# TravisWheelerLab/BATH

Hardware: AMD Instinct MI355X
Metric: DP Gcells/s + residues/s through bathsearch pipeline at 1/2/4/8 MI355X (higher is better)
Workload: dtype u8/i16 integer scores (SSV: exact binary16), f32 Forward

## Files before the change

### bath_amd/csrc/bath_profile.hip

```cpp
#include <atomic>
#include <cctype>
#include <cmath>
#include <cstring>

#include "bath_common.hpp"
#include "host_model.hpp"

using namespace bath;

namespace bath {

static const double kLog2 = 0.69314718055994529;

double gumbel_surv(double x, double mu, double lambda) {
  double ey = -std::exp(-lambda * (x - mu));
  if (std::fabs(ey) < 5e-9) return -ey;
  return 1.0 - std::exp(ey);
}
double gumbel_invsurv(double p, double mu, double lambda) {
  double lp = (p < 5e-9) ? (std::pow(p, p) - 1) / p : std::log(-1. * std::log(1 - p));
  return mu - lp / lambda;
}
double exp_surv(double x, double mu, double lambda) { return (x < mu) ? 1.0 : std::exp(-lambda * (x - mu)); }

// ... 100 lines not shown

extern "C" void bath_hip_finalize(bath_hip_ctx *ctx) {
  if (!ctx) return;
  bath::g_ctx_total.fetch_sub(1);
  if (ctx->internal) bath::g_ctx_internal.fetch_sub(1);
  (void)hipSetDevice(ctx->device);
  (void)hipStreamSynchronize(ctx->stream);
  delete ctx->lane_pool; ctx->lane_pool = nullptr;
  for (bath_hip_ctx *lane : ctx->lanes) bath_hip_finalize(lane);
  ctx->lanes.clear();
  if (ctx->ev_lanes) (void)hipEventDestroy(ctx->ev_lanes);
  if (ctx->aux) { bath_hip_finalize(ctx->aux); ctx->aux = nullptr; }
  if (ctx->aux2) { bath_hip_finalize(ctx->aux2); ctx->aux2 = nullptr; }
  if (ctx->aux3) { bath_hip_finalize(ctx->aux3); ctx->aux3 = nullptr; }
  for (auto &b : ctx->scratch) b.release();
  for (auto &b : ctx->stage) b.release();
  ctx->results_pinned.release();
  for (auto e : ctx->ev_pool) (void)hipEventDestroy(e);
  for (auto e : ctx->span_events) (void)hipEventDestroy(e);
  if (ctx->ev_fork) (void)hipEventDestroy(ctx->ev_fork);
  if (ctx->ev_join) (void)hipEventDestroy(ctx->ev_join);
  if (ctx->copy_stream) (void)hipStreamDestroy(ctx->copy_stream);
  if (ctx->side_stream) (void)hipStreamDestroy(ctx->side_stream);
  (void)hipStreamDestroy(ctx->stream);
  delete ctx;
}

extern "C" int bath_hip_trim(bath_hip_ctx *ctx) {
  if (!ctx) return BATH_EINVAL;
  BATH_HIP_TRY(ctx, hipSetDevice(ctx->device));
  BATH_HIP_TRY(ctx, hipStreamSynchronize(ctx->stream));
  delete ctx->lane_pool; ctx->lane_pool = nullptr;
  for (bath_hip_ctx *lane : ctx->lanes) bath_hip_finalize(lane);
  ctx->lanes.clear();
  if (ctx->aux) { bath_hip_finalize(ctx->aux); ctx->aux = nullptr; }
  if (ctx->aux2) { bath_hip_finalize(ctx->aux2); ctx->aux2 = nullptr; }
  if (ctx->aux3) { bath_hip_finalize(ctx->aux3); ctx->aux3 = nullptr; }
  if (ctx->copy_stream) { (void)hipStreamSynchronize(ctx->copy_stream); (void)hipStreamDestroy(ctx->copy_stream); ctx->copy_stream = nullptr; }
  if (ctx->side_stream) {
    (void)hipStreamSynchronize(ctx->side_stream); (void)hipStreamDestroy(ctx->side_stream); ctx->side_stream = nullptr;
    if (ctx->ev_fork) { (void)hipEventDestroy(ctx->ev_fork); ctx->ev_fork = nullptr; }
    if (ctx->ev_join) { (void)hipEventDestroy(ctx->ev_join); ctx->ev_join = nullptr; }
  }
  ctx->fs_std_orfs.clear(); ctx->fs_std_pool = nullptr; ctx->fs_keep_xoff.clear(); ctx->fs_regions_all.clear();
  ctx->d_records = nullptr; ctx->n_records = 0;
  return BATH_OK;
}

extern "C" const char *bath_hip_last_error(const bath_hip_ctx *ctx) { return ctx ? ctx->err.c_str() : "no context"; }

extern "C" int bath_hip_synchronize(bath_hip_ctx *ctx) {
  BATH_HIP_TRY(ctx, hipSetDevice(ctx->device));
  BATH_HIP_TRY(ctx, hipStreamSynchronize(ctx->stream));
  return BATH_OK;
}

extern "C" void *bath_hip_stream(bath_hip_ctx *ctx) { return (void *)ctx->stream; }
extern "C" int bath_hip_kernel_times(bath_hip_ctx *ctx, int max, bath_kernel_time *out) {
  if (!ctx || !out) return 0;
  int n = 0;
  for (const bath_hip_ctx *c : {(const bath_hip_ctx *)ctx, (const bath_hip_ctx *)ctx->aux, (const bath_hip_ctx *)ctx->aux2, (const bath_hip_ctx *)ctx->aux3}) {
    if (!c) continue;
    for (const bath::KernelSpan &k : c->spans) {
      float ms = 0.f;
      if (hipEventSynchronize(k.b) != hipSuccess || hipEventElapsedTime(&ms, k.a, k.b) != hipSuccess) continue;
      int i = 0;
      while (i < n && out[i].name != k.name) i++;
      if (i == n) { if (n == max) continue; out[n++] = bath_kernel_time{k.name, 0.f, 0, 0.0, 0.0}; }
      out[i].ms += ms; out[i].launches++; out[i].cells += k.cells; out[i].bytes += k.bytes;
    }
  }
  return n;
}
extern "C" int bath_hip_set_fs_serial(bath_hip_ctx *ctx, int on) {
  if (!ctx) return BATH_EINVAL;
  ctx->fs_serial = on < 0 ? -1 : (on ? 1 : 0);
  return BATH_OK;
}

extern "C" int bath_hip_set_fs_strict(bath_hip_ctx *ctx, int on) {
  if (!ctx) return BATH_EINVAL;
  ctx->fs_strict = on ? 1 : 0;
  if (!on && ctx->aux3) { bath_hip_finalize(ctx->aux3); ctx->aux3 = nullptr; }
  for (bath_hip_ctx *l : ctx->lanes) l->fs_strict = ctx->fs_strict;
  return BATH_OK;
}

extern "C" int bath_hip_set_fwd_group(bath_hip_ctx *ctx, int mode) {
  if (!ctx) return BATH_EINVAL;
  if (mode < 0 || mode > 2) { ctx->set_error("bath_hip_set_fwd_group: mode must be 0, 1 or 2"); return BATH_EINVAL; }
  ctx->fwd_group = mode;
  for (bath_hip_ctx *l : ctx->lanes) l->fwd_group = mode;
  return BATH_OK;
}

extern "C" int bath_hip_set_fs_odds(bath_hip_ctx *ctx, int on) {
  if (!ctx) return BATH_EINVAL;
  ctx->fs_odds = on ? 1 : 0;
  for (bath_hip_ctx *l : ctx->lanes) l->fs_odds = ctx->fs_odds;
  return BATH_OK;
}

extern "C" int bath_hip_set_fs5_odds(bath_hip_ctx *ctx, int on) {
  if (!ctx) return BATH_EINVAL;
  ctx->fs5_odds = on ? 1 : 0;
  for (bath_hip_ctx *l : ctx->lanes) l->fs5_odds = ctx->fs5_odds;
  return BATH_OK;
}

extern "C" int bath_hip_set_fs_ensemble(bath_hip_ctx *ctx, int mode) {
  if (!ctx) return BATH_EINVAL;
  if (mode != BATH_ENSEMBLE_SERIAL && mode != BATH_ENSEMBLE_STREAMS_HOST && mode != BATH_ENSEMBLE_STREAMS_DEVICE) { ctx->set_error("bath_hip_set_fs_ensemble: unknown mode " + std::to_string(mode)); return BATH_EINVAL; }
  ctx->fs_ensemble = mode;
  for (bath_hip_ctx *l : ctx->lanes) l->fs_ensemble = mode;
  return BATH_OK;
}

extern "C" int bath_hip_set_std_ensemble(bath_hip_ctx *ctx, int mode) {
  if (!ctx) return BATH_EINVAL;
  if (mode != BATH_ENSEMBLE_SERIAL && mode != BATH_ENSEMBLE_STREAMS_HOST && mode != BATH_ENSEMBLE_STREAMS_DEVICE) { ctx->set_error("bath_hip_set_std_ensemble: unknown mode " + std::to_string(mode)); return BATH_EINVAL; }
  ctx->std_ensemble = mode;
  for (bath_hip_ctx *l : ctx->lanes) l->std_ensemble = mode;
  if (ctx->aux) ctx->aux->std_ensemble = mode;
  return BATH_OK;
}

extern "C" int bath_hip_std_ensemble_counters(bath_hip_ctx *ctx, int64_t *serial_fallbacks, int64_t *twin_fallbacks, int64_t *kernel_regions) {
  if (!ctx) return BATH_EINVAL;
  int64_t s = 0, t = 0, k = 0;
  for (const bath_hip_ctx *c : {(const bath_hip_ctx *)ctx, (const bath_hip_ctx *)ctx->aux}) {
    if (!c) continue;
    s += c->std_ens_serial_fallbacks.load(); t += c->std_ens_twin_fallbacks.load(); k += c->std_ens_kernel_regions.load();
  }
  if (serial_fallbacks) *serial_fallbacks = s;
  if (twin_fallbacks) *twin_fallbacks = t;
  if (kernel_regions) *kernel_regions = k;
  return BATH_OK;
}

extern "C" int bath_hip_fs_ensemble_counters(bath_hip_ctx *ctx, int64_t *bound_fallbacks, int64_t *overflow_fallbacks, int64_t *matrix_bytes_kept) {
  if (!ctx) return BATH_EINVAL;
  int64_t b = 0, o = 0, k = 0;
  for (const bath_hip_ctx *c : {(const bath_hip_ctx *)ctx, (const bath_hip_ctx *)ctx->aux2}) {
    if (!c) continue;
    b += c->fs_ens_bound_fallbacks.load(); o += c->fs_ens_overflow_fallbacks.load(); k += c->fs_ens_bytes_kept.load();
  }
  if (bound_fallbacks) *bound_fallbacks = b;
  if (overflow_fallbacks) *overflow_fallbacks = o;
  if (matrix_bytes_kept) *matrix_bytes_kept = k;
  return BATH_OK;
}

extern "C" int bath_selftest_compute_units(const bath_hip_ctx *ctx) { return ctx ? ctx->prop.multiProcessorCount : 0; }


extern "C" void bath_hip_oprofile_destroy(bath_hip_oprofile *om) {
  if (!om) return;
  for (void *p : {(void *)om->d_emit, (void *)om->d_ssv, (void *)om->d_msv, (void *)om->d_rb, (void *)om->d_rw, (void *)om->d_tw, (void *)om->d_rf, (void *)om->d_tf,
                  (void *)om->d_bias_eo, (void *)om->d_compo_terms, (void *)om->d_vit_rw, (void *)om->d_vit_tw2, (void *)om->d_vit_rank, (void *)om->lt.d_tjb, (void *)om->lt.d_xwmove, (void *)om->lt.d_pmove,
                  (void *)om->lt.d_nullsc, (void *)om->lt.d_lt1, (void *)om->lt.d_lt2, (void *)om->lt.d_p1, (void *)om->d_cons, (void *)om->d_msc, (void *)om->d_tsc, (void *)om->d_rfb, (void *)om->d_tfb})
    if (p) (void)hipFree(p);
  for (void *p : om->retired) (void)hipFree(p);
  delete om;
}

extern "C" int bath_hip_oprofile_set_consensus(bath_hip_oprofile *om, const char *consensus) {
  if (!om || !consensus) return BATH_EINVAL;
  bath_hip_ctx *ctx = om->ctx;
  static const char syms[] = "ACDEFGHIKLMNPQRSTVWY-BJZOUX*~";
  om->consensus.assign((size_t)om->M + 2, ' ');
  om->cons_digital.assign((size_t)om->M + 1, 255);
  for (int k = 1; k <= om->M && consensus[k]; k++) {
    om->consensus[(size_t)k] = consensus[k];
    const char *q = std::strchr(syms, std::toupper((unsigned char)consensus[k]));
    if (q) om->cons_digital[(size_t)k] = (uint8_t)(q - syms);
  }
  if (!om->d_cons) BATH_HIP_TRY(ctx, hipMalloc(&om->d_cons, (size_t)om->M + 1));
  BATH_HIP_TRY(ctx, hipMemcpy(om->d_cons, om->cons_digital.data(), (size_t)om->M + 1, hipMemcpyHostToDevice));
  return BATH_OK;
}

extern "C" int bath_hip_oprofile_M(const bath_hip_oprofile *om) { return om->M; }

extern "C" int bath_hip_oprofile_convert(bath_hip_ctx *ctx, const bath_profile *gm, bath_hip_oprofile **ret) {
  *ret = nullptr;
  const int M = gm->M;
  if (M < 1) { ctx->set_error("profile has no nodes"); return BATH_EINVAL; }
  BATH_HIP_TRY(ctx, hipSetDevice(ctx->device));
  const size_t W = (size_t)M + 1;
  auto msc = [&](int k, int x) { return gm->rsc[(size_t)x * W * 2 + 2 * k]; };
  auto tsc = [&](int k, int s) { return gm->tsc[(size_t)k * 8 + s]; };
  enum { MM, IM, DM, BM, MD, DD, MI, II };

  bath_hip_oprofile *om = new bath_hip_oprofile();
  { static std::atomic<uint64_t> next_uid{1}; om->uid = next_uid.fetch_add(1); }
  om->ctx = ctx; om->M = M; om->max_length = gm->max_length; om->nj = gm->nj; om->L0 = gm->L;
  std::memcpy(om->evparam, gm->evparam, sizeof om->evparam);
  std::memcpy(om->compo, gm->compo, sizeof om->compo);

  float maxsc = 0.0f;
  for (int x = 0; x < 20; x++)
    for (size_t i = 0; i < W * 2; i++) maxsc = std::max(maxsc, gm->rsc[(size_t)x * W * 2 + i]);
  om->scale_b = (float)(3.0 / kLog2);
  om->base_b = 190;
  om->bias_b = cost_u8(om->scale_b, (float)(-1.0 * maxsc));
  om->rb.assign((size_t)kKp * W, 255);
  for (int x = 0; x < kKp; x++)
    for (int k = 1; k <= M; k++) om->rb[x * W + k] = cost_u8_biased(om->scale_b, om->bias_b, msc(k, x));
  om->tbm_b = cost_u8(om->scale_b, logf(2.0f / ((float)M * (float)(M + 1))));
  om->tec_b = cost_u8(om->scale_b, logf(0.5f));

  om->scale_w = (float)(500.0 / kLog2);
  om->base_w = 12000;
  om->rw.assign((size_t)kKp * W, -32768);
  for (int x = 0; x < kKp; x++)
    for (int k = 1; k <= M; k++) om->rw[x * W + k] = score_i16(om->scale_w, msc(k, x));
  om->tw.assign(W * 8, -32768);
  for (int k = 1; k <= M; k++) {
    int16_t *t = &om->tw[(size_t)k * 8];
    for (int s : {BM, MM, IM, DM}) t[s] = std::min<int16_t>(score_i16(om->scale_w, tsc(k - 1, s)), 0);
    for (int s : {MD, MI}) t[s] = (k < M) ? std::min<int16_t>(score_i16(om->scale_w, tsc(k, s)), 0) : (int16_t)-32768;
    t[II] = (k < M) ? std::min<int16_t>(score_i16(om->scale_w, tsc(k, II)), -1) : (int16_t)-32768;
    t[DD] = (k < M) ? score_i16(om->scale_w, tsc(k, DD)) : (int16_t)-32768;
  }
  om->xw_E[0] = score_i16(om->scale_w, gm->xsc[0][0]);
  om->xw_E[1] = score_i16(om->scale_w, gm->xsc[0][1]);
  int ddb = -32768;
  for (int k = 2; k < M - 1; k++)
    ddb = std::max(ddb, (int)score_i16(om->scale_w, tsc(k, DD)) + (int)score_i16(om->scale_w, tsc(k + 1, DM)) -
                            (int)score_i16(om->scale_w, tsc(k + 1, BM)));
  om->ddbound_w = (int16_t)ddb;

  om->rf.assign((size_t)kKp * W, 0.f);
  for (int x = 0; x < kKp; x++)
    for (int k = 1; k <= M; k++) om->rf[x * W + k] = expf(msc(k, x));
  om->tf.assign(W * 8, 0.f);
  for (int k = 1; k <= M; k++) {
    float *t = &om->tf[(size_t)k * 8];
    for (int s : {BM, MM, IM, DM}) t[s] = expf(tsc(k - 1, s));
    for (int s : {MD, MI, II, DD}) t[s] = (k < M) ? expf(tsc(k, s)) : 0.f;
  }
  om->xf_E[0] = expf(gm->xsc[0][0]);
  om->xf_E[1] = expf(gm->xsc[0][1]);

  {
    std::vector<float> &pre = om->prefix_lengths, &suf = om->suffix_lengths;
    pre.assign(W, 0.f); suf.assign(W, 0.f);
    float total = 0;
    for (int k = 1; k < M; k++) {
      const float t_mi = om->tf[(size_t)k * 8 + MI], t_ii = om->tf[(size_t)k * 8 + II];
      pre[k] = (t_mi == 0) ? 1.f : (float)(1 + (int)(std::log(1e-7 / t_mi) / std::log((double)t_ii)));
      total += pre[k];
    }
    pre[0] = pre[M] = 0;
    for (int k = 1; k < M; k++) pre[k] /= total;
    suf[M] = pre[M - 1];
    for (int k = M - 1; k >= 1; k--) suf[k] = suf[k + 1] + pre[k - 1];
    for (int k = 2; k < M; k++) pre[k] += pre[k - 1];
  }

  int G = (M > 152 && M <= 304) ? 2 : 1;
  while (G < 8 && M > 416 * G) G *= 2;
  if (M > 416 * G) { ctx->set_error("model longer than 3328 nodes"); delete om; return BATH_EINVAL; }
  int NR = ((M + G - 1) / G + 1) / 2;
  if (G == 1 && NR <= 112) NR = (NR + 3) / 4 * 4;
  else if (G == 2 && NR <= 76) NR = NR <= 40 ? 40 : (NR <= 72 ? (NR + 7) / 8 * 8 : 76);
  else NR = std::max((NR + 15) / 16 * 16, G > 1 ? 112 : 16);
  NR = std::max(NR, 16);
  om->NR = NR; om->G = G;
  om->ssv_row_bytes = 16 * ((NR * G / 4 + 1) | 1);
  {
    size_t rowsz = (size_t)om->ssv_row_bytes / 2;
    auto half_bits = [](float v) { const _Float16 h = (_Float16)v; int16_t b; std::memcpy(&b, &h, 2); return b; };
    std::vector<int16_t> tab((size_t)kSsvRows * rowsz, half_bits(-1.0f));
    for (int x = 0; x < kKp; x++)
      for (int k = 1; k <= M; k++) {
        const int g = (k - 1) / (2 * NR), q = (k - 1) - g * 2 * NR;
        const int cost = std::min((int)om->rb[x * W + k] - (int)om->bias_b, 127);
        tab[x * rowsz + (size_t)g * 2 * NR + 2 * (q % NR) + q / NR] = half_bits(-(float)cost / 2048.0f);
      }
    BATH_HIP_TRY(ctx, upload(&om->d_ssv, tab.data(), tab.size(), ctx->stream));
    if (G == 1 && NR <= 76) {
      std::vector<int16_t> mtab((size_t)kSsvRows * rowsz, half_bits(-1.0f));
      for (int x = 0; x < kKp; x++)
        for (int k = 1; k <= M; k++) {
          const int q = k - 1;
          const int inc = (int)om->bias_b - (int)om->rb[x * W + k];
          mtab[x * rowsz + 2 * (q % NR) + q / NR] = half_bits((float)inc / 2048.0f);
        }
      BATH_HIP_TRY(ctx, upload(&om->d_msv, mtab.data(), mtab.size(), ctx->stream));
    }
  }
  {
    int NRv = ((M + 1) / 2 + 15) / 16 * 16;
    if (NRv == 80) NRv = std::max(68, ((M + 1) / 2 + 3) / 4 * 4);
    if (NRv <= BATH_TILING_MAX(BATH_VIT_LANE_NR)) {
      om->vit_NR = NRv;
      om->vit_rw_pitch = 4 * NRv + 16;
      const size_t rowsz = (size_t)om->vit_rw_pitch / 2;
      std::vector<int16_t> rwt((size_t)30 * rowsz, (int16_t)-32768);
      auto slot = [&](int node) { return node <= NRv ? 2 * (node - 1) : 2 * (node - NRv - 1) + 1; };
      for (int x = 0; x < kKp; x++)
        for (int k = 1; k <= M; k++) rwt[x * rowsz + slot(k)] = om->rw[x * W + k];
      std::vector<uint32_t> tw2((size_t)NRv * 8);
      std::vector<int16_t> rank((size_t)2 * NRv, (int16_t)32767);
      const int Q8 = std::max(2, ((M - 1) / 8) + 1);
      auto twv = [&](int node, int s) -> int { return node <= M ? (int)om->tw[(size_t)node * 8 + s] : -32768; };
      for (int r = 0; r < NRv; r++)
        for (int s = 0; s < 8; s++) tw2[(size_t)r * 8 + s] = ((uint32_t)(uint16_t)twv(r + 1, s)) | ((uint32_t)(uint16_t)twv(NRv + r + 1, s) << 16);
      for (int node = 1; node <= M; node++) rank[(size_t)slot(node)] = (int16_t)(((node - 1) % Q8) * 8 + (node - 1) / Q8);
      BATH_HIP_TRY(ctx, upload(&om->d_vit_rw, rwt.data(), rwt.size(), ctx->stream));
      BATH_HIP_TRY(ctx, upload(&om->d_vit_tw2, tw2.data(), tw2.size(), ctx->stream));
      BATH_HIP_TRY(ctx, upload(&om->d_vit_rank, rank.data(), rank.size(), ctx->stream));
    }
  }
  om->rb_stride = (int)W;
  BATH_HIP_TRY(ctx, upload(&om->d_rb, om->rb.data(), om->rb.size(), ctx->stream));
  BATH_HIP_TRY(ctx, upload(&om->d_rw, om->rw.data(), om->rw.size(), ctx->stream));
  BATH_HIP_TRY(ctx, upload(&om->d_tw, om->tw.data(), om->tw.size(), ctx->stream));
  BATH_HIP_TRY(ctx, upload(&om->d_rf, om->rf.data(), om->rf.size(), ctx->stream));
  BATH_HIP_TRY(ctx, upload(&om->d_tf, om->tf.data(), om->tf.size(), ctx->stream));
  {
    std::vector<float> tfb((size_t)(M + 2) * 8, 0.f), rfb((size_t)kKp * (M + 2), 0.f);
    std::memcpy(tfb.data(), om->tf.data(), sizeof(float) * (size_t)(M + 1) * 8);
    for (int x = 0; x < kKp; x++) std::memcpy(&rfb[(size_t)x * (M + 2)], &om->rf[(size_t)x * W], sizeof(float) * W);
    BATH_HIP_TRY(ctx, upload(&om->d_tfb, tfb.data(), tfb.size(), ctx->stream));
    BATH_HIP_TRY(ctx, upload(&om->d_rfb, rfb.data(), rfb.size(), ctx->stream));
    BATH_HIP_TRY(ctx, hipStreamSynchronize(ctx->stream));
  }
  {
    std::vector<float> lm((size_t)kKp * W, -INFINITY);
    for (int x = 0; x < kKp; x++)
      for (int k = 1; k <= M; k++) lm[(size_t)x * W + k] = msc(k, x);
    BATH_HIP_TRY(ctx, upload(&om->d_msc, lm.data(), lm.size(), ctx->stream));
    BATH_HIP_TRY(ctx, upload(&om->d_tsc, gm->tsc, (size_t)M * 8, ctx->stream));
    BATH_HIP_TRY(ctx, hipStreamSynchronize(ctx->stream));
  }
  {
    float eo[kKp][2];
    bias_filter_eo(om->compo, eo);
    BATH_HIP_TRY(ctx, upload(&om->d_bias_eo, &eo[0][0], (size_t)kKp * 2, ctx->stream));
  }
  BATH_HIP_TRY(ctx, hipStreamSynchronize(ctx->stream));
  int st = bath::build_compo_terms(ctx, om);
  if (st == BATH_OK) st = om->ensure_len_tables(4096);
  if (st != BATH_OK) { bath_hip_oprofile_destroy(om); return st; }
  *ret = om;
  return BATH_OK;
}

extern "C" int bath_hip_oprofile_scalars(const bath_hip_oprofile *om, int L, bath_oprofile_scalars *o) {
  int st = om->ensure_len_tables(L);
  if (st != BATH_OK) return st;
  o->tbm_b = om->tbm_b; o->tec_b = om->tec_b; o->tjb_b = om->lt.h_tjb[L]; o->base_b = om->base_b; o->bias_b = om->bias_b;
  o->scale_b = om->scale_b;
  o->xw[0][0] = om->xw_E[0]; o->xw[0][1] = om->xw_E[1];
  for (int s = 1; s < 4; s++) { o->xw[s][0] = 0; o->xw[s][1] = om->lt.h_xwmove[L]; }
  o->scale_w = om->scale_w; o->base_w = om->base_w; o->ddbound_w = om->ddbound_w;
  o->xf[0][0] = om->xf_E[0]; o->xf[0][1] = om->xf_E[1];
  for (int s = 1; s < 4; s++) { o->xf[s][1] = om->lt.h_pmove[L]; o->xf[s][0] = 1.0f - om->lt.h_pmove[L]; }
  return BATH_OK;
}

extern "C" int bath_hip_oprofile_get_ssv_scores(const bath_hip_oprofile *om, uint8_t *arr) {
  const size_t W = (size_t)om->M + 1;
  std::memset(arr, 0, W * kKp);
  for (int k = 1; k <= om->M; k++)
    for (int x = 0; x < kKp; x++) arr[(size_t)k * kKp + x] = om->rb[x * W + k];
  return BATH_OK;
}
extern "C" int bath_hip_oprofile_get_vit(const bath_hip_oprofile *om, int16_t *rw, int16_t *tw) {
  std::memcpy(rw, om->rw.data(), om->rw.size() * sizeof(int16_t));
  std::memcpy(tw, om->tw.data(), om->tw.size() * sizeof(int16_t));
  return BATH_OK;
}
extern "C" int bath_hip_oprofile_get_fwd(const bath_hip_oprofile *om, float *rf, float *tf) {
  std::memcpy(rf, om->rf.data(), om->rf.size() * sizeof(float));
  std::memcpy(tf, om->tf.data(), om->tf.size() * sizeof(float));
  return BATH_OK;
}


extern "C" void bath_hip_seqs_destroy(bath_hip_seqs *sq) {
  if (!sq) return;
  for (bath_hip_seqs *part : sq->parts) bath_hip_seqs_destroy(part);
  sq->parts.clear();
  if (sq->is_part) { sq->d_data = nullptr; sq->d_len = nullptr; sq->d_context = nullptr; }
  for (void *p : {(void *)sq->d_data, (void *)sq->d_off, (void *)sq->d_len, (void *)sq->d_context, (void *)sq->d_tile_desc, (void *)sq->d_tile_first,
                  (void *)sq->d_packed, (void *)sq->d_poff, sq->d_exc})
    if (p) (void)hipFree(p);
  if (sq->ev_upload) (void)hipEventDestroy(sq->ev_upload);
  delete sq;
}

extern "C" int64_t bath_hip_seqs_count(const bath_hip_seqs *sq) { return sq->n; }

extern "C" int64_t bath_hip_seqs_read(const bath_hip_seqs *sq, uint8_t *data, int64_t cap, int64_t *offsets, int32_t *lengths, int32_t *context) {
  if (!sq || cap < 0 || (cap > 0 && !data)) return -1;
  bath_hip_ctx *ctx = sq->ctx;
  const int64_t bytes = sq->total_aligned + 64;
  if (hipSetDevice(ctx->device) != hipSuccess || hipStreamSynchronize(ctx->stream) != hipSuccess) { ctx->set_error("seqs_read: the block's stream failed"); return -1; }
  auto get = [&](void *dst, const void *src, size_t n) { return n == 0 || !dst || hipMemcpy(dst, src, n, hipMemcpyDeviceToHost) == hipSuccess; };
  const bool ok = get(data, sq->d_data, (size_t)std::min(cap, bytes)) && get(offsets, sq->d_off, (size_t)sq->n * sizeof(int64_t)) &&
                  get(lengths, sq->d_len, (size_t)sq->n * sizeof(int32_t)) &&
                  (!context || (sq->d_context ? get(context, sq->d_context, (size_t)sq->n * sizeof(int32_t)) : (std::memset(context, 0, (size_t)sq->n * sizeof(int32_t)), true)));
  if (!ok) { ctx->set_error("seqs_read: copy to the host failed"); return -1; }
  return bytes;
}

extern "C" int bath_hip_seqs_set_context(bath_hip_seqs *sq, const int32_t *context) {
  if (!sq || sq->is_part) return BATH_EINVAL;
  bath_hip_ctx *ctx = sq->ctx;
  BATH_HIP_TRY(ctx, hipSetDevice(ctx->device));
  for (bath_hip_seqs *part : sq->parts) bath_hip_seqs_destroy(part);
  sq->parts.clear();
  sq->cache_minlen = -1;
  if (!context) { if (sq->d_context) (void)hipFree(sq->d_context); sq->d_context = nullptr; sq->h_context.clear(); return BATH_OK; }
  for (int64_t i = 0; i < sq->n; i++) if (context[i] < 0 || context[i] > sq->h_len[(size_t)i]) { ctx->set_error("context longer than its window"); return BATH_EINVAL; }
  sq->h_context.assign(context, context + sq->n);
  if (!sq->d_context) BATH_HIP_TRY(ctx, hipMalloc((void **)&sq->d_context, (size_t)std::max<int64_t>(sq->n, 1) * sizeof(int32_t)));
  if (sq->n > 0) BATH_HIP_TRY(ctx, hipMemcpy(sq->d_context, sq->h_context.data(), (size_t)sq->n * sizeof(int32_t), hipMemcpyHostToDevice));
  return BATH_OK;
}

extern "C" int bath_hip_seqs_create(bath_hip_ctx *ctx, const uint8_t *dsq, const int64_t *offsets, int64_t n, bath_hip_seqs **ret) {
  *ret = nullptr;
  if (n < 0) return BATH_EINVAL;
  BATH_HIP_TRY(ctx, hipSetDevice(ctx->device));
  bath_hip_seqs *sq = new bath_hip_seqs();
  sq->ctx = ctx; sq->n = n;
  sq->h_off.resize(n); sq->h_len.resize(n);
  int64_t pos = 0;
  bool contiguous_ok = true;
  for (int64_t i = 0; i < n; i++) {
    int64_t L = offsets[i + 1] - offsets[i];
    if (L < 0 || L > INT32_MAX) { delete sq; ctx->set_error("bad sequence offsets"); return BATH_EINVAL; }
    sq->h_off[i] = pos; sq->h_len[i] = (int32_t)L;
    if (pos != offsets[i] - offsets[0]) contiguous_ok = false;
    sq->maxlen = std::max(sq->maxlen, (int32_t)L);
    sq->total += L;
    pos += (L + 15) / 16 * 16;
  }
  sq->total_aligned = pos;
  size_t bytes = (size_t)pos + 64;
  BATH_HIP_TRY(ctx, hipMalloc((void **)&sq->d_data, bytes));
  BATH_HIP_TRY(ctx, hipMalloc((void **)&sq->d_off, (size_t)std::max<int64_t>(n, 1) * sizeof(int64_t)));
  BATH_HIP_TRY(ctx, hipMalloc((void **)&sq->d_len, (size_t)std::max<int64_t>(n, 1) * sizeof(int32_t)));
  BATH_HIP_TRY(ctx, hipMemsetAsync(sq->d_data, 0x1d, bytes, ctx->stream));
  std::vector<uint8_t> staged;
  if (n > 0) {
    if (contiguous_ok) {
      BATH_HIP_TRY(ctx, hipMemcpyAsync(sq->d_data, dsq + offsets[0], (size_t)(offsets[n] - offsets[0]), hipMemcpyHostToDevice, ctx->stream));
    } else {
      staged.assign((size_t)pos, 0x1d);
      for (int64_t i = 0; i < n; i++) std::memcpy(staged.data() + sq->h_off[i], dsq + offsets[i], (size_t)sq->h_len[i]);
      BATH_HIP_TRY(ctx, hipMemcpyAsync(sq->d_data, staged.data(), staged.size(), hipMemcpyHostToDevice, ctx->stream));
    }
    BATH_HIP_TRY(ctx, hipMemcpyAsync(sq->d_off, sq->h_off.data(), (size_t)n * sizeof(int64_t), hipMemcpyHostToDevice, ctx->stream));
    BATH_HIP_TRY(ctx, hipMemcpyAsync(sq->d_len, sq->h_len.data(), (size_t)n * sizeof(int32_t), hipMemcpyHostToDevice, ctx->stream));
  }
  BATH_HIP_TRY(ctx, hipStreamSynchronize(ctx->stream));
  *ret = sq;
  return BATH_OK;
}


namespace {
struct ExcRec { int64_t seq; int32_t pos, code; };

__global__ __launch_bounds__(256) void unpack2_kernel(const uint8_t *__restrict__ packed, const int64_t *__restrict__ poff, const int64_t *__restrict__ off,
                                                      const int32_t *__restrict__ len, uint8_t *__restrict__ data, int64_t n) {
  const int64_t s = (int64_t)blockIdx.x * 4 + (threadIdx.x >> 6);
  if (s >= n) return;
  const int lane = threadIdx.x & 63;
  const int L = len[s];
  const int nb = (L + 3) >> 2;
  const uint8_t *src = packed + poff[s];
  uint8_t *dst = data + off[s];
  const int j_lo = blockIdx.y * 4096, j_hi = min((nb + 3) >> 2, j_lo + 4096);
  for (int j = j_lo + lane; j < j_hi; j += 64) {
    uint32_t w;
    if (4 * j + 4 <= nb) w = *reinterpret_cast<const uint32_t *>(src + 4 * j);
    else { w = 0; for (int q = 0; 4 * j + q < nb; q++) w |= (uint32_t)src[4 * j + q] << (8 * q); }
    uint32_t v[4];
#pragma unroll
    for (int q = 0; q < 4; q++) {
      const unsigned b = (w >> (8 * q)) & 0xffu;
      v[q] = (b & 3u) | ((b >> 2) & 3u) << 8 | ((b >> 4) & 3u) << 16 | ((b >> 6) & 3u) << 24;
    }
    if (16 * j + 16 <= L) *reinterpret_cast<uint4 *>(dst + 16 * j) = make_uint4(v[0], v[1], v[2], v[3]);
    else for (int q = 0; 16 * j + q < L; q++) dst[16 * j + q] = (uint8_t)((v[q >> 2] >> (8 * (q & 3))) & 0xffu);
  }
}
__global__ void unpack_exceptions_kernel(const ExcRec *__restrict__ exc, int64_t n, const int64_t *__restrict__ off, uint8_t *__restrict__ data) {
  const int64_t i = (int64_t)blockIdx.x * blockDim.x + threadIdx.x;
  if (i < n) data[off[exc[i].seq] + exc[i].pos] = (uint8_t)exc[i].code;
}
}

extern "C" void *bath_hip_host_alloc(size_t bytes) {
  void *p = nullptr;
  return hipHostMalloc(&p, bytes ? bytes : 1, hipHostMallocDefault) == hipSuccess ? p : nullptr;
}
extern "C" void bath_hip_host_free(void *p) { if (p) (void)hipHostFree(p); }

extern "C" int bath_hip_seqs_create_packed(bath_hip_ctx *ctx, const int64_t *offsets, int64_t n, bath_hip_seqs **ret) {
  *ret = nullptr;
  if (!ctx || !offsets || n < 0) return BATH_EINVAL;
  std::vector<uint8_t> zeros((size_t)std::max<int64_t>(offsets[n] - offsets[0], 1), 0);
  std::vector<int64_t> rel((size_t)n + 1);
  for (int64_t i = 0; i <= n; i++) rel[(size_t)i] = offsets[i] - offsets[0];
  bath_hip_seqs *sq = nullptr;
  int st = bath_hip_seqs_create(ctx, zeros.data(), rel.data(), n, &sq);
  if (st != BATH_OK) return st;
  std::vector<int64_t> poff((size_t)n + 1, 0);
  for (int64_t i = 0; i < n; i++) poff[(size_t)i + 1] = poff[(size_t)i] + (sq->h_len[(size_t)i] + 3) / 4;
  sq->packed_bytes = poff[(size_t)n];
  auto packed_parts = [&]() -> int {
    BATH_HIP_TRY(ctx, hipMalloc((void **)&sq->d_packed, (size_t)sq->packed_bytes + 64));
    BATH_HIP_TRY(ctx, hipMalloc((void **)&sq->d_poff, (size_t)(n + 1) * sizeof(int64_t)));
    BATH_HIP_TRY(ctx, hipMemcpy(sq->d_poff, poff.data(), (size_t)(n + 1) * sizeof(int64_t), hipMemcpyHostToDevice));
    BATH_HIP_TRY(ctx, hipEventCreateWithFlags(&sq->ev_upload, hipEventDisableTiming));
    return BATH_OK;
  };
  if ((st = packed_parts()) != BATH_OK) { bath_hip_seqs_destroy(sq); return st; }
  *ret = sq;
  return BATH_OK;
}

extern "C" int bath_hip_seqs_upload_packed(bath_hip_seqs *sq, const uint8_t *packed, const int64_t *exc_seq, const int32_t *exc_pos,
                                           const uint8_t *exc_code, int64_t n_exc) {
  if (!sq || !sq->d_packed || !packed || n_exc < 0) return BATH_EINVAL;
  bath_hip_ctx *ctx = sq->ctx;
  BATH_HIP_TRY(ctx, hipSetDevice(ctx->device));
  if (!ctx->copy_stream) BATH_HIP_TRY(ctx, hipStreamCreateWithFlags(&ctx->copy_stream, hipStreamNonBlocking));
  if (n_exc > sq->exc_cap) {
    if (sq->d_exc) (void)hipFree(sq->d_exc);
    sq->exc_cap = n_exc + n_exc / 2 + 1024;
    BATH_HIP_TRY(ctx, hipMalloc(&sq->d_exc, (size_t)sq->exc_cap * sizeof(ExcRec)));
  }
  BATH_HIP_TRY(ctx, hipMemcpyAsync(sq->d_packed, packed, (size_t)sq->packed_bytes, hipMemcpyHostToDevice, ctx->copy_stream));
  if (n_exc > 0) {
    std::vector<ExcRec> h((size_t)n_exc);
    for (int64_t i = 0; i < n_exc; i++) {
      if (exc_seq[i] < 0 || exc_seq[i] >= sq->n || exc_pos[i] < 0 || exc_pos[i] >= sq->h_len[(size_t)exc_seq[i]]) { ctx->set_error("exception outside its sequence"); return BATH_EINVAL; }
      h[(size_t)i] = ExcRec{exc_seq[i], exc_pos[i], (int32_t)exc_code[i]};
    }
    BATH_HIP_TRY(ctx, hipMemcpyAsync(sq->d_exc, h.data(), (size_t)n_exc * sizeof(ExcRec), hipMemcpyHostToDevice, ctx->copy_stream));
    BATH_HIP_TRY(ctx, hipStreamSynchronize(ctx->copy_stream));
  }
  sq->n_exc = n_exc;
  BATH_HIP_TRY(ctx, hipEventRecord(sq->ev_upload, ctx->copy_stream));
  sq->upload_pending = true;
  return BATH_OK;
}

extern "C" int bath_hip_seqs_upload_wait(bath_hip_seqs *sq) {
  if (!sq || !sq->d_packed) return BATH_EINVAL;
  if (!sq->upload_pending) return BATH_OK;
  bath_hip_ctx *ctx = sq->ctx;
  BATH_HIP_TRY(ctx, hipSetDevice(ctx->device));
  BATH_HIP_TRY(ctx, hipStreamWaitEvent(ctx->stream, sq->ev_upload, 0));
  if (sq->n > 0) {
    const unsigned gy = (unsigned)std::max(1, ((sq->maxlen + 15) / 16 + 4095) / 4096);
    hipLaunchKernelGGL(unpack2_kernel, dim3((unsigned)((sq->n + 3) / 4), gy), dim3(256), 0, ctx->stream, sq->d_packed, sq->d_poff, sq->d_off, sq->d_len, sq->d_data, sq->n);
    if (sq->n_exc > 0)
      hipLaunchKernelGGL(unpack_exceptions_kernel, dim3((unsigned)((sq->n_exc + 255) / 256)), dim3(256), 0, ctx->stream, (const ExcRec *)sq->d_exc, sq->n_exc, sq->d_off, sq->d_data);
    BATH_HIP_TRY(ctx, hipGetLastError());
  }
  hipEvent_t ev = sq->ev_upload;
  BATH_HIP_TRY(ctx, hipEventRecord(ev, ctx->stream));
  for (bath_hip_ctx *l : ctx->lanes) BATH_HIP_TRY(ctx, hipStreamWaitEvent(l->stream, ev, 0));
  sq->upload_pending = false;
  return BATH_OK;
}
```

### bath_amd/csrc/bath_viterbi.hip

```cpp
#include <algorithm>
#include <cstdlib>
#include <functional>

#include "bath_common.hpp"
#include "bath_kernels.hpp"
#include "bath_launch.hpp"

using namespace bath;

namespace bath {

__device__ __forceinline__ s16x2 pk_adds(s16x2 a, s16x2 b) { return __builtin_elementwise_add_sat(a, b); }
__device__ __forceinline__ s16x2 pk_max(s16x2 a, s16x2 b) { return __builtin_elementwise_max(a, b); }
__device__ __forceinline__ s16x2 as_s2(unsigned v) { return __builtin_bit_cast(s16x2, v); }
__device__ __forceinline__ unsigned as_u(s16x2 v) { return __builtin_bit_cast(unsigned, v); }

struct VitLaneTables {
  const int16_t *rw;
  int rw_pitch_bytes;
  const uint32_t *tw2;
  const int16_t *rank;
};

struct VitLaneConsts {
  int M, base_w, xwE_loop, xwE_move, Q8;
  float scale_w;
  double invP_vit, invP_msv;
  float scale_b;
  int base_b, tec_b, bias_b;
};

typedef uint32_t u32x16 __attribute__((ext_vector_type(16)));

template <int NR>
__global__ __launch_bounds__(256, 1) void vit_lane_kernel(SeqView sq, VitLaneTables tb, const uint32_t *__restrict__ tw2g, VitLaneConsts c, const int16_t *__restrict__ xwmove_tab,
                                                          const uint8_t *__restrict__ tjb_tab, const int32_t *__restrict__ todo, int64_t ntodo,
                                                          const int *__restrict__ ntodo_dev, const int *__restrict__ skip_dev, float *__restrict__ sc, int32_t *__restrict__ status,
                                                          const float *__restrict__ filtersc, const uint8_t *__restrict__ ssv_scores,
                                                          WindowRec *__restrict__ wins, int *__restrict__ win_count, int win_cap, int32_t *__restrict__ kminmax) {
  extern __shared__ __attribute__((aligned(16))) char lds[];
  char *s_rw = lds;
  int16_t *s_rank = reinterpret_cast<int16_t *>(lds + 30 * tb.rw_pitch_bytes);
  {
    const uint32_t *src = reinterpret_cast<const uint32_t *>(tb.rw);
    uint32_t *dst = reinterpret_cast<uint32_t *>(s_rw);
    for (int i = threadIdx.x; i < 30 * tb.rw_pitch_bytes / 4; i += blockDim.x) dst[i] = src[i];
    for (int i = threadIdx.x; i < 2 * NR; i += blockDim.x) s_rank[i] = tb.rank[i];
  }
  __syncthreads();
  if (ntodo_dev) ntodo = *ntodo_dev;
  const int64_t t = (int64_t)blockIdx.x * blockDim.x + threadIdx.x + (skip_dev ? *skip_dev : 0);
  if (t - (threadIdx.x & 63) >= ntodo) return;
  const bool live = t < ntodo;
  const int64_t sid = live ? (todo ? (int64_t)todo[t] : t) : (todo ? (int64_t)todo[0] : 0);
  const int L = live ? sq.len[sid] : 0;
  const uint8_t *s = sq.data + sq.off[sid];
  const int Lw = wave_max_i32(L);
  const bool do_win = (wins != nullptr);
  const int M = c.M;

  const int xw_move = xwmove_tab[L];
  int sc_thresh = 0, sc_ext_thresh = 0, skip_until = 0, kmin = 1 << 30, kmax = 0;
  if (do_win && live) {
    const double fsc = (double)filtersc[sid];
    sc_thresh = (int)(int16_t)(int)ceil(((fsc + 0.69314718055994529 * c.invP_vit + 3.0) * (double)c.scale_w) -
                                        (double)(float)c.xwE_move - (double)(float)xw_move + (double)(float)c.base_w);
    sc_ext_thresh = (int)ceil(((fsc + 0.69314718055994529 * c.invP_msv + 3.0) * (double)c.scale_b) + c.base_b + c.tec_b + (int)tjb_tab[L]);
  }
  const s16x2 NEG = {-32768, -32768};
  s16x2 Mr[NR], Ir[NR], Dr[NR];
#pragma unroll
  for (int r = 0; r < NR; r++) Mr[r] = Ir[r] = Dr[r] = NEG;
  int xN = c.base_w;
  int xB = (int16_t)(xN + xw_move);
  int xJ = -32768, xC = -32768;
  bool overflow = false;
  short ePrev = -32768;

  uint32_t wnext = (0 < L) ? *reinterpret_cast<const uint32_t *>(s) : 0x1d1d1d1du;
  for (int i0 = 0; i0 < Lw; i0 += 4) {
    const uint32_t w = wnext;
    wnext = (i0 + 4 < L) ? *reinterpret_cast<const uint32_t *>(s + i0 + 4) : 0x1d1d1d1du;
#pragma unroll 1
    for (int j = 0; j < 4; j++) {
      const int i = i0 + j + 1;
      const bool on = (i <= L) && !overflow;
      int x = (w >> (8 * j)) & 0xff;
      x = (i <= L) ? min(x, kKp - 1) : 29;
      const char *rowbase = s_rw + x * tb.rw_pitch_bytes;
      const s16x2 xBv = {(short)xB, (short)xB};
      s16x2 xEv = NEG;
      unsigned pM = (as_u(Mr[NR - 1]) << 16) | 0x8000u, pI = (as_u(Ir[NR - 1]) << 16) | 0x8000u, pD = (as_u(Dr[NR - 1]) << 16) | 0x8000u;
      s16x2 dpk = NEG;
      s16x2 cpk = {(short)-32768, ePrev};
      int twz = 0;
      asm volatile("" : "+s"(twz));
      const uint32_t *tw = tw2g + twz;
      u32x16 t_c, t_n;
      int4 e_c = *reinterpret_cast<const int4 *>(rowbase), e_n = e_c;
      asm volatile("s_load_dwordx16 %0, %1, 0x0" : "=s"(t_c) : "s"(tw));
#pragma unroll
      for (int r = 0; r < NR; r += 2) {
        asm volatile("s_waitcnt lgkmcnt(0)" ::: "memory");
        __builtin_amdgcn_sched_barrier(0);
        if ((r & 3) == 0 && r + 4 < NR) e_n = *reinterpret_cast<const int4 *>(rowbase + 4 * (r + 4));
        if (r + 2 < NR) asm volatile("s_load_dwordx16 %0, %1, %2" : "=s"(t_n) : "s"(tw), "i"((r + 2) * 32));
        __builtin_amdgcn_sched_barrier(0);
        const unsigned em[2] = {(r & 3) ? (unsigned)e_c.z : (unsigned)e_c.x, (r & 3) ? (unsigned)e_c.w : (unsigned)e_c.y};
#pragma unroll
        for (int q = 0; q < 2; q++) {
          const int rr = r + q;
          const unsigned tMM = t_c[8 * q + 0], tIM = t_c[8 * q + 1], tDM = t_c[8 * q + 2], tBM = t_c[8 * q + 3];
          const unsigned tMD = t_c[8 * q + 4], tDD = t_c[8 * q + 5], tMI = t_c[8 * q + 6], tII = t_c[8 * q + 7];
          const unsigned oM = as_u(Mr[rr]), oI = as_u(Ir[rr]);
          const unsigned oD = as_u(pk_max(Dr[rr], cpk));
          cpk = pk_adds(cpk, as_s2(tDD));
          const s16x2 ms = as_s2(pM), is = as_s2(pI), ds = as_s2(pD);
          s16x2 sv = pk_adds(xBv, as_s2(tBM));
          sv = pk_max(sv, pk_adds(ms, as_s2(tMM)));
          sv = pk_max(sv, pk_adds(is, as_s2(tIM)));
          sv = pk_max(sv, pk_adds(ds, as_s2(tDM)));
          sv = pk_adds(sv, as_s2(em[q]));
          Ir[rr] = pk_max(pk_adds(as_s2(oM), as_s2(tMI)), pk_adds(as_s2(oI), as_s2(tII)));
          const s16x2 dcv = pk_adds(sv, as_s2(tMD));
          xEv = pk_max(xEv, sv);
          Mr[rr] = sv;
          Dr[rr] = dpk;
          dpk = pk_max(dcv, pk_adds(dpk, as_s2(tDD)));
          pM = oM; pI = oI; pD = oD;
        }
        if (r + 2 < NR) t_c = t_n;
        if ((r & 3) == 2 && r + 2 < NR) e_c = e_n;
        asm volatile("" : "+v"(Mr[r]), "+v"(Mr[r + 1]), "+v"(Ir[r]), "+v"(Ir[r + 1]), "+v"(Dr[r]), "+v"(Dr[r + 1]), "+v"(dpk), "+v"(cpk), "+v"(xEv));
        __builtin_amdgcn_sched_barrier(0);
      }
      ePrev = dpk.x;
      if (on) {
        const int xE = max((int)xEv.x, (int)xEv.y);
        if (xE >= 32767) overflow = true;
        else {
          xN = (int16_t)(xN + 0);
          xC = (int16_t)max(xC + 0, xE + c.xwE_move);
          xJ = (int16_t)max(xJ + 0, xE + c.xwE_loop);
          xB = (int16_t)max(xJ + xw_move, xN + xw_move);
          if (do_win && i > skip_until && xE >= sc_thresh) {
            int rank = 32767;
#pragma unroll
            for (int r = 0; r < NR; r++) {
              if ((int)Mr[r].x == xE) rank = min(rank, (int)s_rank[2 * r]);
              if ((int)Mr[r].y == xE) rank = min(rank, (int)s_rank[2 * r + 1]);
            }
            const int k_start = (rank / 8) + c.Q8 * (rank % 8) + 1;
            int max_k_end = k_start, max_i_end = i, sc_ext = sc_ext_thresh, max_sc_ext = sc_ext, since = 0;
            int kk = k_start + 1, nn = i + 1;
            while (kk <= M && nn <= L) {
              sc_ext += c.bias_b - (int)ssv_scores[(size_t)kk * kKp + min((int)s[nn - 1], kKp - 1)];
              if (sc_ext >= max_sc_ext) { max_sc_ext = sc_ext; max_k_end = kk; max_i_end = nn; since = 0; }
              else if (++since == 5) break;
              kk++; nn++;
            }
            const int slot = atomicAdd(win_count, 1);
            if (slot < win_cap) wins[slot] = WindowRec{(int32_t)sid, i, max_k_end, max_k_end - k_start + 1, 0.0f};
            kmax = max(kmax, max_k_end);
            kmin = min(kmin, k_start);
            skip_until = max_i_end;
          }
        }
      }
    }
  }
  if (live) {
    if (overflow) { sc[sid] = INFINITY; status[sid] = BATH_ERANGE; }
    else if (xC > -32768) {
      float r = (float)xC + (float)xw_move - (float)c.base_w;
      r /= c.scale_w;
      r = (float)((double)r - 3.0);
      sc[sid] = r; status[sid] = BATH_OK;
    } else { sc[sid] = -INFINITY; status[sid] = BATH_OK; }
    if (do_win && kminmax) { kminmax[2 * sid] = kmin; kminmax[2 * sid + 1] = kmax; }
  }
}

constexpr int kLenBins = 2048;
constexpr int kVitLongTarget = 128;
__device__ __forceinline__ void len_block_range(int n, int &lo, int &hi) {
  const int per = (n + (int)gridDim.x - 1) / (int)gridDim.x;
  lo = min(n, (int)blockIdx.x * per); hi = min(n, lo + per);
}
__global__ __launch_bounds__(256) void len_hist_kernel(const int32_t *__restrict__ todo, const int *__restrict__ ntodo_dev, const int32_t *__restrict__ len,
                                                       int *__restrict__ hist) {
  __shared__ int s_cnt[kLenBins];
  for (int i = threadIdx.x; i < kLenBins; i += blockDim.x) s_cnt[i] = 0;
  __syncthreads();
  int lo, hi;
  len_block_range(*ntodo_dev, lo, hi);
  for (int j = lo + threadIdx.x; j < hi; j += blockDim.x) atomicAdd(&s_cnt[min(len[todo[j]], kLenBins - 1)], 1);
  __syncthreads();
  for (int i = threadIdx.x; i < kLenBins; i += blockDim.x) if (s_cnt[i]) atomicAdd(&hist[i], s_cnt[i]);
}
__global__ __launch_bounds__(256) void len_scan_kernel(int *__restrict__ hist ) {
  constexpr int kPer = kLenBins / 256;
  __shared__ int s_wsum[4];
  const int tid = threadIdx.x, lane = tid & 63, wv = tid >> 6;
  int c[kPer], sum = 0;
#pragma unroll
  for (int k = 0; k < kPer; k++) { c[k] = hist[kLenBins - 1 - (kPer * tid + k)]; sum += c[k]; }
  int x = sum;
#pragma unroll
  for (int d = 1; d < 64; d <<= 1) { const int y = __shfl_up(x, d, 64); if (lane >= d) x += y; }
  if (lane == 63) s_wsum[wv] = x;
  __syncthreads();
  int run = x - sum;
#pragma unroll
  for (int u = 0; u < 4; u++) run += u < wv ? s_wsum[u] : 0;
#pragma unroll
  for (int k = 0; k < kPer; k++) { hist[kLenBins - 1 - (kPer * tid + k)] = run; run += c[k]; }
}
__global__ __launch_bounds__(256) void len_scatter_kernel(const int32_t *__restrict__ todo, const int *__restrict__ ntodo_dev, const int32_t *__restrict__ len,
                                                          int *__restrict__ cursor, int32_t *__restrict__ sorted) {
  __shared__ int s_cnt[kLenBins];
  for (int i = threadIdx.x; i < kLenBins; i += blockDim.x) s_cnt[i] = 0;
  __syncthreads();
  int lo, hi;
  len_block_range(*ntodo_dev, lo, hi);
  for (int j = lo + threadIdx.x; j < hi; j += blockDim.x) atomicAdd(&s_cnt[min(len[todo[j]], kLenBins - 1)], 1);
  __syncthreads();
  for (int i = threadIdx.x; i < kLenBins; i += blockDim.x) { const int c = s_cnt[i]; if (c) s_cnt[i] = atomicAdd(&cursor[i], c); }
  __syncthreads();
  for (int j = lo + threadIdx.x; j < hi; j += blockDim.x) {
    const int cnd = todo[j];
    sorted[atomicAdd(&s_cnt[min(len[cnd], kLenBins - 1)], 1)] = cnd;
  }
}

int vit_lane_supported(const bath_hip_oprofile *om) { return om->vit_NR > 0; }

const int *len_sort_count_longer(const int *d_bins, int T) { return d_bins + std::min(T + 1, kLenBins - 1); }

int launch_len_sort(bath_hip_ctx *ctx, const int32_t *d_todo, const int *d_ntodo, const int32_t *d_len, int *d_bins, int32_t *d_sorted) {
  BATH_HIP_TRY(ctx, hipMemsetAsync(d_bins, 0, kLenBins * sizeof(int), ctx->stream));
  hipLaunchKernelGGL(len_hist_kernel, dim3(256), dim3(256), 0, ctx->stream, d_todo, d_ntodo, d_len, d_bins);
  hipLaunchKernelGGL(len_scan_kernel, dim3(1), dim3(256), 0, ctx->stream, d_bins);
  hipLaunchKernelGGL(len_scatter_kernel, dim3(256), dim3(256), 0, ctx->stream, d_todo, d_ntodo, d_len, d_bins, d_sorted);
  BATH_HIP_TRY(ctx, hipGetLastError());
  return BATH_OK;
}

extern "C" int bath_selftest_len_sort(bath_hip_ctx *ctx, int n, const int32_t *lens, int T, int32_t *sorted, int32_t *n_longer) {
  if (!ctx || n < 0 || (n > 0 && (!lens || !sorted)) || !n_longer) return BATH_EINVAL;
  BATH_HIP_TRY(ctx, hipSetDevice(ctx->device));
  const size_t m = (size_t)std::max(n, 1);
  int32_t *d = nullptr;
  BATH_HIP_TRY(ctx, hipMalloc((void **)&d, (3 * m + kLenBins + 1) * sizeof(int32_t)));
  int32_t *d_len = d, *d_todo = d + m, *d_sorted = d + 2 * m, *d_bins = d + 3 * m, *d_n = d_bins + kLenBins;
  std::vector<int32_t> todo(m);
  for (size_t i = 0; i < m; i++) todo[i] = (int32_t)i;
  hipError_t e = hipSuccess;
  if (n > 0) e = hipMemcpy(d_len, lens, (size_t)n * sizeof(int32_t), hipMemcpyHostToDevice);
  if (e == hipSuccess) e = hipMemcpy(d_todo, todo.data(), m * sizeof(int32_t), hipMemcpyHostToDevice);
  if (e == hipSuccess) e = hipMemcpy(d_n, &n, sizeof(int32_t), hipMemcpyHostToDevice);
  int st = e == hipSuccess ? launch_len_sort(ctx, d_todo, d_n, d_len, d_bins, d_sorted) : BATH_EFAIL;
  if (st == BATH_OK) e = hipStreamSynchronize(ctx->stream);
  if (st == BATH_OK && e == hipSuccess && n > 0) e = hipMemcpy(sorted, d_sorted, (size_t)n * sizeof(int32_t), hipMemcpyDeviceToHost);
  if (st == BATH_OK && e == hipSuccess) e = hipMemcpy(n_longer, len_sort_count_longer(d_bins, T), sizeof(int32_t), hipMemcpyDeviceToHost);
  (void)hipFree(d);
  if (st == BATH_OK && e != hipSuccess) { ctx->set_error(std::string("bath_selftest_len_sort: ") + hipGetErrorString(e)); st = BATH_EFAIL; }
  return st;
}

int launch_vit_lane(bath_hip_ctx *ctx, const bath_hip_oprofile *om, SeqView v, const int32_t *d_todo, int64_t ntodo, const int *ntodo_dev,
                    float *d_sc, int32_t *d_status, const VitWindowArgs *wa, const int *skip_dev) {
  if (ntodo == 0) return BATH_OK;
  VitLaneTables tb{om->d_vit_rw, om->vit_rw_pitch, om->d_vit_tw2, om->d_vit_rank};
  VitLaneConsts c{};
  c.M = om->M; c.base_w = om->base_w; c.xwE_loop = om->xw_E[0]; c.xwE_move = om->xw_E[1]; c.Q8 = std::max(2, ((om->M - 1) / 8) + 1);
  c.scale_w = om->scale_w; c.scale_b = om->scale_b; c.base_b = om->base_b; c.tec_b = om->tec_b; c.bias_b = om->bias_b;
  const float *fsc = nullptr; const uint8_t *ssv = nullptr; WindowRec *wins = nullptr; int *wc = nullptr; int cap = 0; int32_t *kmm = nullptr;
  if (wa) { c.invP_vit = wa->invP_vit; c.invP_msv = wa->invP_msv; fsc = wa->d_filtersc; ssv = wa->d_ssv_scores; wins = (WindowRec *)wa->d_wins; wc = wa->d_win_count; cap = wa->win_cap; kmm = wa->d_kminmax; }
  const int NRv = om->vit_NR;
  const size_t shmem = (size_t)30 * om->vit_rw_pitch + (size_t)2 * NRv * 2 + 16;
  const int blocks = (int)((ntodo + 255) / 256);
  bool launched = false;
#define BATH_VITL_CASE(N, ...)                                                                                                         \
  if (!launched && NRv == N) {                                                                                                         \
    hipLaunchKernelGGL(vit_lane_kernel<N>, dim3(blocks), dim3(256), shmem, ctx->stream, v, tb, tb.tw2, c, om->lt.d_xwmove, om->lt.d_tjb, d_todo, ntodo, \
                       ntodo_dev, skip_dev, d_sc, d_status, fsc, ssv, wins, wc, cap, kmm);                                                       \
    launched = true;                                                                                                                   \
  }
  BATH_VIT_LANE_NR(BATH_VITL_CASE)
#undef BATH_VITL_CASE
  if (!launched) { ctx->set_error("lane-per-target Viterbi kernel: unsupported model length"); return BATH_EINVAL; }
  BATH_HIP_TRY(ctx, hipGetLastError());
  return BATH_OK;
}

int64_t lane_min_nt() {
  static const int64_t v = [] { const char *e = std::getenv("BATH_HIP_LANE_MIN_NT"); return e ? std::atoll(e) : (int64_t)150'000'000; }();
  return v;
}

const char *vit_lane_kernel_name(const bath_hip_oprofile *om) {
#define BATH_VITL_NAME(N, ...) if (om->vit_NR == N) return "vit_lane_kernel<" #N ">";
  BATH_VIT_LANE_NR(BATH_VITL_NAME)
#undef BATH_VITL_NAME
  return "vit_lane_kernel<?>";
}

int launch_vit_sorted(bath_hip_ctx *ctx, const bath_hip_oprofile *om, SeqView v, const int32_t *d_todo, int64_t cap, const int *d_ntodo, const int32_t *d_len,
                      int *d_bins, int32_t *d_sorted, float *d_sc, int32_t *d_status, const VitWindowArgs *wa, const std::function<int(hipStream_t)> &beside) {
  int st;
  if ((st = launch_len_sort(ctx, d_todo, d_ntodo, d_len, d_bins, d_sorted)) != BATH_OK) return st;
  if (!ctx->side_stream) {
    BATH_HIP_TRY(ctx, hipStreamCreateWithFlags(&ctx->side_stream, hipStreamNonBlocking));
    BATH_HIP_TRY(ctx, hipEventCreateWithFlags(&ctx->ev_fork, hipEventDisableTiming));
    BATH_HIP_TRY(ctx, hipEventCreateWithFlags(&ctx->ev_join, hipEventDisableTiming));
  }
  const int *d_nlong = len_sort_count_longer(d_bins, kVitLongTarget);
  BATH_HIP_TRY(ctx, hipEventRecord(ctx->ev_fork, ctx->stream));
  BATH_HIP_TRY(ctx, hipStreamWaitEvent(ctx->side_stream, ctx->ev_fork, 0));
  {
    hipStream_t main_stream = ctx->stream;
    ctx->stream = ctx->side_stream;
    st = launch_vit_wave(ctx, om, v, d_sorted, cap, d_sc, d_status, wa, d_nlong);
    ctx->stream = main_stream;
    if (st != BATH_OK) return st;
    if (beside && (st = beside(ctx->side_stream)) != BATH_OK) return st;
  }
  BATH_HIP_TRY(ctx, hipEventRecord(ctx->ev_join, ctx->side_stream));
  if ((st = launch_vit_lane(ctx, om, v, d_sorted, cap, d_ntodo, d_sc, d_status, wa, d_nlong)) != BATH_OK) return st;
  BATH_HIP_TRY(ctx, hipStreamWaitEvent(ctx->stream, ctx->ev_join, 0));
  return BATH_OK;
}

}
```

Measured before the change: 215.3 billion.

## Precompute next-row M/I/D transition max in Viterbi lane kernel via shifted table layout

```diff
diff --git a/bath_amd/csrc/bath_profile.hip b/bath_amd/csrc/bath_profile.hip
--- a/bath_amd/csrc/bath_profile.hip
+++ b/bath_amd/csrc/bath_profile.hip
@@ -426,12 +426,13 @@
       auto slot = [&](int node) { return node <= NRv ? 2 * (node - 1) : 2 * (node - NRv - 1) + 1; };
       for (int x = 0; x < kKp; x++)
         for (int k = 1; k <= M; k++) rwt[x * rowsz + slot(k)] = om->rw[x * W + k];
-      std::vector<uint32_t> tw2((size_t)NRv * 8);
+      std::vector<uint32_t> tw2((size_t)(NRv + 1) * 8, 0x80008000u);
       std::vector<int16_t> rank((size_t)2 * NRv, (int16_t)32767);
       const int Q8 = std::max(2, ((M - 1) / 8) + 1);
       auto twv = [&](int node, int s) -> int { return node <= M ? (int)om->tw[(size_t)node * 8 + s] : -32768; };
       for (int r = 0; r < NRv; r++)
-        for (int s = 0; s < 8; s++) tw2[(size_t)r * 8 + s] = ((uint32_t)(uint16_t)twv(r + 1, s)) | ((uint32_t)(uint16_t)twv(NRv + r + 1, s) << 16);
+        for (int s = 0; s < 8; s++)
+          tw2[(size_t)(s < BM ? (r > 0 ? r - 1 : NRv) : r) * 8 + s] =((uint32_t)(uint16_t)twv(r + 1, s)) | ((uint32_t)(uint16_t)twv(NRv + r + 1, s) << 16);
       for (int node = 1; node <= M; node++) rank[(size_t)slot(node)] = (int16_t)(((node - 1) % Q8) * 8 + (node - 1) / Q8);
       BATH_HIP_TRY(ctx, upload(&om->d_vit_rw, rwt.data(), rwt.size(), ctx->stream));
       BATH_HIP_TRY(ctx, upload(&om->d_vit_tw2, tw2.data(), tw2.size(), ctx->stream));
diff --git a/bath_amd/csrc/bath_viterbi.hip b/bath_amd/csrc/bath_viterbi.hip
--- a/bath_amd/csrc/bath_viterbi.hip
+++ b/bath_amd/csrc/bath_viterbi.hip
@@ -31,6 +31,7 @@
 };
 
 typedef uint32_t u32x16 __attribute__((ext_vector_type(16)));
+typedef uint32_t u32x4 __attribute__((ext_vector_type(4)));
 
 template <int NR>
 __global__ __launch_bounds__(256, 1) void vit_lane_kernel(SeqView sq, VitLaneTables tb, const uint32_t *__restrict__ tw2g, VitLaneConsts c, const int16_t *__restrict__ xwmove_tab,
@@ -81,8 +82,9 @@
   for (int i0 = 0; i0 < Lw; i0 += 4) {
     const uint32_t w = wnext;
     wnext = (i0 + 4 < L) ? *reinterpret_cast<const uint32_t *>(s + i0 + 4) : 0x1d1d1d1du;
+    const int nj = min(4, Lw - i0);
 #pragma unroll 1
-    for (int j = 0; j < 4; j++) {
+    for (int j = 0; j < nj; j++) {
       const int i = i0 + j + 1;
       const bool on = (i <= L) && !overflow;
       int x = (w >> (8 * j)) & 0xff;
@@ -90,15 +92,20 @@
       const char *rowbase = s_rw + x * tb.rw_pitch_bytes;
       const s16x2 xBv = {(short)xB, (short)xB};
       s16x2 xEv = NEG;
-      unsigned pM = (as_u(Mr[NR - 1]) << 16) | 0x8000u, pI = (as_u(Ir[NR - 1]) << 16) | 0x8000u, pD = (as_u(Dr[NR - 1]) << 16) | 0x8000u;
-      s16x2 dpk = NEG;
+      const unsigned pM = (as_u(Mr[NR - 1]) << 16) | 0x8000u, pI = (as_u(Ir[NR - 1]) << 16) | 0x8000u, pD = (as_u(Dr[NR - 1]) << 16) | 0x8000u;
       s16x2 cpk = {(short)-32768, ePrev};
       int twz = 0;
       asm volatile("" : "+s"(twz));
       const uint32_t *tw = tw2g + twz;
       u32x16 t_c, t_n;
+      u32x4 t_0;
       int4 e_c = *reinterpret_cast<const int4 *>(rowbase), e_n = e_c;
+      asm volatile("s_load_dwordx4 %0, %1, %2" : "=s"(t_0) : "s"(tw), "i"(NR * 32));
       asm volatile("s_load_dwordx16 %0, %1, 0x0" : "=s"(t_c) : "s"(tw));
+      asm volatile("s_waitcnt lgkmcnt(0)" : "+s"(t_0) : : "memory");
+      s16x2 pre =pk_max(pk_max(pk_adds(as_s2(pM), as_s2(t_0[0])), pk_adds(as_s2(pI), as_s2(t_0[1]))), pk_adds(as_s2(pD), as_s2(t_0[2])));
+      s16x2 oD = pk_max(Dr[0], cpk);
+      Dr[0] = NEG;
 #pragma unroll
       for (int r = 0; r < NR; r += 2) {
         asm volatile("s_waitcnt lgkmcnt(0)" ::: "memory");
@@ -110,31 +117,29 @@
 #pragma unroll
         for (int q = 0; q < 2; q++) {
           const int rr = r + q;
-          const unsigned tMM = t_c[8 * q + 0], tIM = t_c[8 * q + 1], tDM = t_c[8 * q + 2], tBM = t_c[8 * q + 3];
+          const unsigned nMM = t_c[8 * q + 0], nIM = t_c[8 * q + 1], nDM = t_c[8 * q + 2], tBM = t_c[8 * q + 3];
           const unsigned tMD = t_c[8 * q + 4], tDD = t_c[8 * q + 5], tMI = t_c[8 * q + 6], tII = t_c[8 * q + 7];
-          const unsigned oM = as_u(Mr[rr]), oI = as_u(Ir[rr]);
-          const unsigned oD = as_u(pk_max(Dr[rr], cpk));
+          const s16x2 oM = Mr[rr], oI = Ir[rr];
           cpk = pk_adds(cpk, as_s2(tDD));
-          const s16x2 ms = as_s2(pM), is = as_s2(pI), ds = as_s2(pD);
-          s16x2 sv = pk_adds(xBv, as_s2(tBM));
-          sv = pk_max(sv, pk_adds(ms, as_s2(tMM)));
-          sv = pk_max(sv, pk_adds(is, as_s2(tIM)));
-          sv = pk_max(sv, pk_adds(ds, as_s2(tDM)));
+          s16x2 sv = pk_max(pk_adds(xBv, as_s2(tBM)), pre);
+          if (rr + 1 < NR) pre = pk_max(pk_max(pk_adds(oM, as_s2(nMM)), pk_adds(oI, as_s2(nIM))), pk_adds(oD, as_s2(nDM)));
+          Ir[rr] = pk_max(pk_adds(oM, as_s2(tMI)), pk_adds(oI, as_s2(tII)));
+          asm volatile("" : "+v"(sv), "+v"(pre), "+v"(Ir[rr]));
           sv = pk_adds(sv, as_s2(em[q]));
-          Ir[rr] = pk_max(pk_adds(as_s2(oM), as_s2(tMI)), pk_adds(as_s2(oI), as_s2(tII)));
-          const s16x2 dcv = pk_adds(sv, as_s2(tMD));
+          s16x2 dcv = pk_adds(sv, as_s2(tMD));
           xEv = pk_max(xEv, sv);
           Mr[rr] = sv;
-          Dr[rr] = dpk;
-          dpk = pk_max(dcv, pk_adds(dpk, as_s2(tDD)));
-          pM = oM; pI = oI; pD = oD;
+          if (rr + 1 < NR) {
+            oD = pk_max(Dr[rr + 1], cpk);
+            asm volatile("" : "+v"(oD), "+v"(dcv));
+            Dr[rr + 1] = pk_max(dcv, pk_adds(Dr[rr], as_s2(tDD)));
+          } else ePrev = pk_max(dcv, pk_adds(Dr[rr], as_s2(tDD))).x;
         }
         if (r + 2 < NR) t_c = t_n;
         if ((r & 3) == 2 && r + 2 < NR) e_c = e_n;
-        asm volatile("" : "+v"(Mr[r]), "+v"(Mr[r + 1]), "+v"(Ir[r]), "+v"(Ir[r + 1]), "+v"(Dr[r]), "+v"(Dr[r + 1]), "+v"(dpk), "+v"(cpk), "+v"(xEv));
+        asm volatile("" : "+v"(Mr[r]), "+v"(Mr[r + 1]), "+v"(Ir[r]), "+v"(Ir[r + 1]), "+v"(Dr[r + 1]), "+v"(Dr[r + 2 < NR ? r + 2 : r]), "+v"(oD), "+v"(cpk), "+v"(xEv), "+v"(pre));
         __builtin_amdgcn_sched_barrier(0);
       }
-      ePrev = dpk.x;
       if (on) {
         const int xE = max((int)xEv.x, (int)xEv.y);
         if (xE >= 32767) overflow = true;
```

After: 214.6 billion (median of 2 runs). No clear change (-0.3%).
